# AlexandreRouma/SDRPlusPlus

Measured on AMD Instinct MI355X. Metric: IQ Msamples/s ingested (65536-pt FFT + 32 VFO WFM), higher is better.
Workload: dtype f32

## Files before the change

include/sdrpp_gpu.h:

```cpp
#ifndef SDRPP_GPU_H
#define SDRPP_GPU_H

#include <stddef.h>
#include <stdint.h>

#ifdef __cplusplus
extern "C" {
#endif

#define SDRPP_OK 0
#define SDRPP_ERR_NO_DEVICE (-1)
#define SDRPP_ERR_INVALID (-2)
#define SDRPP_ERR_NOMEM (-3)
#define SDRPP_ERR_HIP (-4)
#define SDRPP_ERR_UNSUPPORTED (-5)
#define SDRPP_ERR_NOT_FOUND (-6)

typedef struct sdrpp_ctx sdrpp_ctx;

int sdrpp_device_count(void);
int sdrpp_create(int device, int64_t max_push, sdrpp_ctx** ctx);
int sdrpp_destroy(sdrpp_ctx* ctx);
const char* sdrpp_strerror(int code);
const char* sdrpp_last_error(const sdrpp_ctx* ctx);
// ... 196 lines not shown
} sdrpp_iq_format;
int sdrpp_push_raw(sdrpp_ctx* ctx, const void* iq_host, int64_t count, const sdrpp_iq_format* fmt);
int sdrpp_push_frame(sdrpp_ctx* ctx, const unsigned char* frame, int bytes, int* samples);
int sdrpp_design_u8_table(int source, float gain, float* table256);
int sdrpp_abi_sizeof_iq_format(void);

void* sdrpp_host_alloc(size_t bytes);
void sdrpp_host_free(void* p);
void* sdrpp_device_alloc(sdrpp_ctx* ctx, size_t bytes);
void sdrpp_device_free(sdrpp_ctx* ctx, void* p);
int sdrpp_device_copy(sdrpp_ctx* ctx, void* dst, const void* src, size_t bytes, int kind);
int sdrpp_set_deferred(sdrpp_ctx* ctx, int on);
int sdrpp_push_pinned_async(sdrpp_ctx* ctx, const float* iq_pinned, int64_t count);
int sdrpp_push_wait(sdrpp_ctx* ctx);
int64_t sdrpp_pending(sdrpp_ctx* ctx);

int sdrpp_push_stage(sdrpp_ctx* ctx, int64_t count, float** slot);
int sdrpp_push_staged(sdrpp_ctx* ctx, int64_t count);
int sdrpp_push_staged_when(sdrpp_ctx* ctx, int64_t count, const volatile uint32_t* pending);
#define SDRPP_RESULT_SLOTS 24
#define SDRPP_GROUP_MAX 32
typedef struct sdrpp_result {
    uint64_t ticket;
    int n_vfo;
    const int* ids;
    const int64_t* offsets;
    const int* counts;
    const float* samples;
    int n_lines, fft_size, data_width;
    const float* zoomed;
    const int32_t* index;
    const float* raw;
    int n_iq;
    const float* iq;
} sdrpp_result;
int sdrpp_set_pipelined(sdrpp_ctx* ctx, int on, int result_flags);
int sdrpp_result_rec(sdrpp_ctx* ctx, uint64_t ticket, int id, const void** data, sdrpp_rec_info* info);
#define SDRPP_RESULT_RDS 32
int sdrpp_pipeline_set_rds_results(sdrpp_ctx* ctx, int on);
int sdrpp_result_rds(sdrpp_ctx* ctx, uint64_t ticket, int id, const float** data, int* count);
int sdrpp_result_meters(sdrpp_ctx* ctx, uint64_t ticket, const float** data, int* n_lines, int* n_meters);
int sdrpp_set_pipeline_group(sdrpp_ctx* ctx, int max_blocks, int adaptive);
int sdrpp_pipeline_launch_held(sdrpp_ctx* ctx);
int sdrpp_pipeline_group_stats(sdrpp_ctx* ctx, int64_t* out, int max);
uint64_t sdrpp_ticket(sdrpp_ctx* ctx);
int sdrpp_pipeline_flush(sdrpp_ctx* ctx);
int sdrpp_result_ready(sdrpp_ctx* ctx, uint64_t ticket);
int sdrpp_result_wait(sdrpp_ctx* ctx, uint64_t ticket, sdrpp_result* out);
int sdrpp_result_release(sdrpp_ctx* ctx, uint64_t ticket);
int sdrpp_result_take_lines(sdrpp_ctx* ctx, uint64_t ticket, float* zoomed_dst, int32_t* index_dst, int max_lines, int* n_lines);
#define SDRPP_PIPELINE_STATS_HEAD 8
int sdrpp_pipeline_stats(sdrpp_ctx* ctx, int64_t* out, int max);
const char* sdrpp_pipeline_role_name(int role);
int sdrpp_pass_form_stats(sdrpp_ctx* ctx, int64_t* out, const char** names, int max);

#define SDRPP_NUM_KERNEL_FAMILIES 13
int sdrpp_timing_enable(sdrpp_ctx* ctx, int on);
int sdrpp_timing_read(sdrpp_ctx* ctx, double* ms_per_family, int64_t* launches_per_family);
const char* sdrpp_kernel_family_name(int family);

#ifdef __cplusplus
}
#endif
#endif
```

sdrplusplus_amd/capi.py:

```python
import ctypes as C
import os

import numpy as np

_HERE = os.path.dirname(os.path.abspath(__file__))
DEFAULT_LIB = os.path.join(_HERE, "csrc", "libsdrpp_gpu.so")

MAX_DECIM_STAGES = 4
NUM_KERNEL_FAMILIES = 13

DEMOD_RAW, DEMOD_WFM, DEMOD_NFM, DEMOD_AM, DEMOD_USB, DEMOD_LSB, DEMOD_DSB, DEMOD_CW = -1, 0, 1, 2, 3, 4, 5, 6

c_float_p = C.POINTER(C.c_float)
c_int_p = C.POINTER(C.c_int)
c_int32_p = C.POINTER(C.c_int32)


class VfoDesc(C.Structure):

    _fields_ = [
        ("phase_delta_re", C.c_float),
        ("phase_delta_im", C.c_float),
        ("n_stages", C.c_int),
        ("stage_decim", C.c_int * MAX_DECIM_STAGES),
# ... 265 lines not shown
    L.sdrpp_vfo_remove.argtypes = [vp, C.c_int]
    L.sdrpp_vfo_replace.argtypes = [vp, C.c_int, C.POINTER(VfoDesc), C.c_int, c_int_p]
    L.sdrpp_vfo_count.argtypes = [vp]
    L.sdrpp_vfo_set_phase_delta.argtypes = [vp, C.c_int, C.c_float, C.c_float]
    L.sdrpp_vfo_set_channel_taps.argtypes = [vp, C.c_int, c_float_p, C.c_int]
    L.sdrpp_vfo_reset.argtypes = [vp, C.c_int]
    L.sdrpp_set_reference_block.argtypes = [vp, C.c_int]
    L.sdrpp_set_deferred.argtypes = [vp, C.c_int]
    L.sdrpp_push_pinned_async.argtypes = [vp, c_float_p, C.c_int64]
    L.sdrpp_push_wait.argtypes = [vp]
    L.sdrpp_push_stage.argtypes = [vp, C.c_int64, C.POINTER(c_float_p)]
    L.sdrpp_push_staged.argtypes = [vp, C.c_int64]
    L.sdrpp_push_staged_when.argtypes = [vp, C.c_int64, C.POINTER(C.c_uint32)]
    L.sdrpp_host_alloc.restype = vp
    L.sdrpp_host_alloc.argtypes = [C.c_size_t]
    L.sdrpp_host_free.restype = None
    L.sdrpp_host_free.argtypes = [vp]
    L.sdrpp_device_alloc.restype = vp
    L.sdrpp_device_alloc.argtypes = [vp, C.c_size_t]
    L.sdrpp_device_free.restype = None
    L.sdrpp_device_free.argtypes = [vp, vp]
    L.sdrpp_device_copy.restype = C.c_int
    L.sdrpp_device_copy.argtypes = [vp, vp, vp, C.c_size_t, C.c_int]
    L.sdrpp_pending.restype = C.c_int64
    L.sdrpp_pending.argtypes = [vp]
    L.sdrpp_vfo_read_many.argtypes = [vp, C.c_int, c_int_p, c_int_p, c_float_p, C.c_int64, C.POINTER(C.c_int64), c_int_p]
    L.sdrpp_set_nco_mode.argtypes = [vp, C.c_int]
    L.sdrpp_set_backend_pipeline.argtypes = [vp, C.c_int]
    L.sdrpp_vfo_set_ssb_phase_delta.argtypes = [vp, C.c_int, C.c_float, C.c_float]
    L.sdrpp_vfo_out_count.argtypes = [vp, C.c_int]
    L.sdrpp_vfo_read.argtypes = [vp, C.c_int, c_float_p, C.c_int]
    L.sdrpp_vfo_device_buffers.argtypes = [vp, C.c_int, C.POINTER(vp), c_int_p, C.POINTER(vp), c_int_p]
    L.sdrpp_push.argtypes = [vp, c_float_p, C.c_int64]
    L.sdrpp_push_device.argtypes = [vp, vp, C.c_int64]
    L.sdrpp_push_int16.argtypes = [vp, C.POINTER(C.c_int16), C.c_int64]
    L.sdrpp_abi_sizeof_iq_format.argtypes = []
    if L.sdrpp_abi_sizeof_iq_format() != C.sizeof(IqFormat):
        raise ImportError("sdrpp_iq_format layout mismatch: library %d bytes, binding %d" % (L.sdrpp_abi_sizeof_iq_format(), C.sizeof(IqFormat)))
    L.sdrpp_push_raw.argtypes = [vp, vp, C.c_int64, C.POINTER(IqFormat)]
    L.sdrpp_push_frame.argtypes = [vp, C.c_char_p, C.c_int, c_int_p]
    L.sdrpp_design_u8_table.argtypes = [C.c_int, C.c_float, c_float_p]
    L.sdrpp_set_pipelined.argtypes = [vp, C.c_int, C.c_int]
    L.sdrpp_set_pipeline_group.argtypes = [vp, C.c_int, C.c_int]
    L.sdrpp_pipeline_group_stats.argtypes = [vp, C.POINTER(C.c_int64), C.c_int]
    L.sdrpp_ticket.restype = C.c_uint64
    L.sdrpp_ticket.argtypes = [vp]
    L.sdrpp_pipeline_flush.argtypes = [vp]
    L.sdrpp_pipeline_launch_held.argtypes = [vp]
    L.sdrpp_result_ready.argtypes = [vp, C.c_uint64]
    L.sdrpp_result_wait.argtypes = [vp, C.c_uint64, C.POINTER(Result)]
    L.sdrpp_result_release.argtypes = [vp, C.c_uint64]
    L.sdrpp_result_take_lines.argtypes = [vp, C.c_uint64, vp, vp, C.c_int, c_int_p]
    L.sdrpp_pipeline_stats.argtypes = [vp, C.POINTER(C.c_int64), C.c_int]
    L.sdrpp_pipeline_role_name.restype = C.c_char_p
    L.sdrpp_pipeline_role_name.argtypes = [C.c_int]
    L.sdrpp_pass_form_stats.argtypes = [vp, C.POINTER(C.c_int64), C.POINTER(C.c_char_p), C.c_int]
    L.sdrpp_timing_enable.argtypes = [vp, C.c_int]
    L.sdrpp_timing_read.argtypes = [vp, C.POINTER(C.c_double), C.POINTER(C.c_int64)]
    L.sdrpp_kernel_family_name.restype = C.c_char_p
    L.sdrpp_kernel_family_name.argtypes = [C.c_int]
    _lib, _lib_path = L, path
    return L


EXPORTED_SYMBOLS = [
    "sdrpp_create", "sdrpp_destroy", "sdrpp_strerror", "sdrpp_last_error", "sdrpp_set_stream", "sdrpp_sync", "sdrpp_abi_version", "sdrpp_device_info",
    "sdrpp_design_low_pass", "sdrpp_design_high_pass", "sdrpp_design_fft_window", "sdrpp_design_reshape_params",
    "sdrpp_design_phase_delta", "sdrpp_design_resampler", "sdrpp_design_waterfall_view", "sdrpp_design_deemphasis_alpha",
    "sdrpp_vfo_read_pcm", "sdrpp_vfo_read_compressed", "sdrpp_preproc_read_pcm",
    "sdrpp_wf_configure", "sdrpp_wf_set_smoothing", "sdrpp_wf_set_hold", "sdrpp_wf_latest", "sdrpp_wf_raster", "sdrpp_wf_signal_info",
    "sdrpp_wf_set_meters", "sdrpp_wf_meters_read", "sdrpp_result_meters", "sdrpp_abi_sizeof_meter_desc",
    "sdrpp_preproc_configure", "sdrpp_preproc_reconfigure", "sdrpp_preproc_set_reference_order", "sdrpp_preproc_out_count", "sdrpp_preproc_read", "sdrpp_preproc_device_buffer",
    "sdrpp_vfo_set_rec", "sdrpp_vfo_rec_read", "sdrpp_abi_sizeof_rec_desc", "sdrpp_result_rec",
    "sdrpp_vfo_set_rds", "sdrpp_vfo_rds_count", "sdrpp_vfo_rds_read", "sdrpp_vfo_rds_device_buffer", "sdrpp_abi_sizeof_rds_desc", "sdrpp_rds_bank_count",
    "sdrpp_pipeline_set_rds_results", "sdrpp_result_rds",
    "sdrpp_vfo_set_stereo", "sdrpp_abi_sizeof_stereo_desc", "sdrpp_design_band_pass_complex", "sdrpp_design_pll",
    "sdrpp_vfo_set_af", "sdrpp_vfo_af_count", "sdrpp_vfo_af_read", "sdrpp_vfo_af_device_buffer", "sdrpp_abi_sizeof_af_desc",
    "sdrpp_vfo_set_if", "sdrpp_vfo_set_fmnr", "sdrpp_vfo_ifc_count", "sdrpp_vfo_ifc_read", "sdrpp_vfo_ifc_device_buffer", "sdrpp_abi_sizeof_if_desc",
    "sdrpp_fft_configure", "sdrpp_fft_disable", "sdrpp_fft_set_view", "sdrpp_fft_lines", "sdrpp_fft_read", "sdrpp_fft_copy_device", "sdrpp_fft_device_buffers",
    "sdrpp_vfo_add", "sdrpp_vfo_remove", "sdrpp_vfo_replace", "sdrpp_vfo_count", "sdrpp_vfo_set_phase_delta", "sdrpp_vfo_set_channel_taps", "sdrpp_vfo_reset",
    "sdrpp_vfo_out_count", "sdrpp_vfo_read", "sdrpp_vfo_device_buffers",
    "sdrpp_set_reference_block", "sdrpp_set_nco_mode", "sdrpp_set_backend_pipeline", "sdrpp_vfo_set_ssb_phase_delta", "sdrpp_vfo_read_many", "sdrpp_set_deferred", "sdrpp_push_pinned_async", "sdrpp_push_wait", "sdrpp_pending", "sdrpp_host_alloc", "sdrpp_host_free", "sdrpp_device_alloc", "sdrpp_device_free", "sdrpp_device_copy", "sdrpp_device_count",
    "sdrpp_push_raw", "sdrpp_push_frame", "sdrpp_design_u8_table", "sdrpp_abi_sizeof_iq_format",
    "sdrpp_push", "sdrpp_push_device", "sdrpp_push_int16", "sdrpp_push_stage", "sdrpp_push_staged", "sdrpp_push_staged_when",
    "sdrpp_set_pipelined", "sdrpp_set_pipeline_group", "sdrpp_pipeline_group_stats", "sdrpp_ticket", "sdrpp_pipeline_flush", "sdrpp_pipeline_launch_held", "sdrpp_result_ready", "sdrpp_result_wait", "sdrpp_result_release", "sdrpp_result_take_lines", "sdrpp_pipeline_stats", "sdrpp_pipeline_role_name", "sdrpp_pass_form_stats",
    "sdrpp_timing_enable", "sdrpp_timing_read", "sdrpp_kernel_family_name",
]


def pass_form_names():
    names = (C.c_char_p * 128)()
    n = load().sdrpp_pass_form_stats(None, None, names, 128)
    return [names[i].decode() for i in range(n)]


def design_low_pass(cutoff, trans_width, sample_rate, odd=False):
    L = load()
    n = L.sdrpp_design_low_pass(cutoff, trans_width, sample_rate, int(odd), None, 0)
    taps = np.zeros(max(n, 1), dtype=np.float32)
    L.sdrpp_design_low_pass(cutoff, trans_width, sample_rate, int(odd), taps.ctypes.data_as(c_float_p), n)
    return taps[:n]


def design_high_pass(cutoff, trans_width, sample_rate, odd=False):
    L = load()
    n = L.sdrpp_design_high_pass(cutoff, trans_width, sample_rate, int(odd), None, 0)
    taps = np.zeros(max(n, 1), dtype=np.float32)
    L.sdrpp_design_high_pass(cutoff, trans_width, sample_rate, int(odd), taps.ctypes.data_as(c_float_p), n)
    return taps[:n]


def design_band_pass_complex(band_start, band_stop, trans_width, sample_rate, odd=False):
    L = load()
    n = L.sdrpp_design_band_pass_complex(band_start, band_stop, trans_width, sample_rate, int(odd), None, 0)
    if n <= 0:
        raise SdrppError(n, "sdrpp_design_band_pass_complex")
    taps = np.empty(n, dtype=np.complex64)
    L.sdrpp_design_band_pass_complex(band_start, band_stop, trans_width, sample_rate, int(odd), taps.view(np.float32).ctypes.data_as(c_float_p), 2 * n)
    return taps


def design_pll(bandwidth):
    a, b = C.c_float(), C.c_float()
    load().sdrpp_design_pll(bandwidth, C.byref(a), C.byref(b))
    return a.value, b.value


def design_fft_window(kind, nz):
    w = np.empty(nz, dtype=np.float32)
    rc = load().sdrpp_design_fft_window(kind, nz, w.ctypes.data_as(c_float_p))
    if rc:
        raise SdrppError(rc, "bad window parameters")
    return w


def design_reshape_params(sample_rate, fft_size, fft_rate):
    skip, nz = C.c_int(), C.c_int()
    load().sdrpp_design_reshape_params(sample_rate, fft_size, fft_rate, C.byref(skip), C.byref(nz))
# ... 458 lines not shown
    def push_staged_from(self, iq):
        iq = np.ascontiguousarray(iq, dtype=np.complex64)
        slot = c_float_p()
        self._chk(self.L.sdrpp_push_stage(self.h, len(iq), C.byref(slot)))
        C.memmove(slot, iq.ctypes.data, len(iq) * 8)
        self._chk(self.L.sdrpp_push_staged(self.h, len(iq)))

    def push_staged_late_fill(self, iq, delay_s=0.002):
        import threading
        import time

        iq = np.ascontiguousarray(iq, dtype=np.complex64)
        slot = c_float_p()
        self._chk(self.L.sdrpp_push_stage(self.h, len(iq), C.byref(slot)))
        pending = C.c_uint32(2)
        dst = C.cast(slot, C.c_void_p).value
        half = (len(iq) // 2) * 8

        def fill():
            time.sleep(delay_s)
            C.memmove(dst, iq.ctypes.data, half)
            pending.value = 1
            time.sleep(delay_s)
            C.memmove(dst + half, iq.ctypes.data + half, len(iq) * 8 - half)
            pending.value = 0

        th = threading.Thread(target=fill)
        th.start()
        try:
            self._chk(self.L.sdrpp_push_staged_when(self.h, len(iq), C.byref(pending)))
        finally:
            th.join()

    def result_lines_into(self, ticket, dst_addr, max_lines):
        n = self._take_n
        rc = self.L.sdrpp_result_take_lines(self.h, ticket, dst_addr, None, max_lines, n)
        if rc < 0:
            self._chk(rc)
        return self._take_n_val.value

    def result_release(self, ticket):
        self._chk(self.L.sdrpp_result_release(self.h, int(ticket)))

    def pipeline_stats(self):
        buf = (C.c_int64 * 128)()
        n = self._chk(self.L.sdrpp_pipeline_stats(self.h, buf, 128))
        nroles = int(buf[5])
        roles = {}
        for r in range(nroles):
            if 8 + r < n and buf[8 + r]:
                roles[self.L.sdrpp_pipeline_role_name(r).decode()] = int(buf[8 + r])
        return dict(ticks=int(buf[0]), tick_blocks=int(buf[1]), pass_blocks=int(buf[2]), crowded_ticks=int(buf[3]), depth=int(buf[4]), table_bytes=int(buf[7]), roles=roles)

    def pass_form_stats(self):
        buf = (C.c_int64 * 128)()
        names = (C.c_char_p * 128)()
        n = self._chk(self.L.sdrpp_pass_form_stats(self.h, buf, names, 128))
        return {names[i].decode(): int(buf[i]) for i in range(n) if buf[i]}

    def timing_enable(self, on=True, families=None):
        v = int(bool(on))
        if on and families is not None:
            mask = 0
            for f in families:
                mask |= 1 << int(f)
            v = (1 | (mask << 1)) if mask else 0
        self._chk(self.L.sdrpp_timing_enable(self.h, v))

    def family_index(self, name):
        for i in range(NUM_KERNEL_FAMILIES):
            if self.L.sdrpp_kernel_family_name(i).decode() == name:
                return i
        raise KeyError(name)

    def timing_read(self):
        ms = (C.c_double * NUM_KERNEL_FAMILIES)()
        ln = (C.c_int64 * NUM_KERNEL_FAMILIES)()
        self._chk(self.L.sdrpp_timing_read(self.h, ms, ln))
        return {self.L.sdrpp_kernel_family_name(i).decode(): (ms[i], ln[i]) for i in range(NUM_KERNEL_FAMILIES)}


_hip = None


def _copy_from_device(L, host_ptr, dev_ptr, nbytes):
    global _hip
    if "emu" in os.path.basename(lib_path()):
        C.memmove(host_ptr, dev_ptr, nbytes)
        return
    if _hip is None:
        _hip = C.CDLL("libamdhip64.so")
        _hip.hipMemcpy.argtypes = [C.c_void_p, C.c_void_p, C.c_size_t, C.c_int]
    rc = _hip.hipMemcpy(C.c_void_p(host_ptr), C.c_void_p(dev_ptr), nbytes, 2)
    if rc:
        raise SdrppError(-4, "hipMemcpy D2H failed (%d)" % rc)
```

sdrplusplus_amd/csrc/host_ctx.h:

```cpp
#pragma once

namespace {

constexpr int kArenaSlots = 24;
constexpr size_t kArenaBytes = 4u << 20;
constexpr int kRing = 4;
constexpr int kTickDepth = 18;
constexpr int kResSlots = SDRPP_RESULT_SLOTS;
constexpr int kGroupMax = SDRPP_GROUP_MAX;
constexpr int kResMeta = kResSlots * kGroupMax;
constexpr int kStageSlots = 4;
constexpr int kChanMaxTaps = 65536;
constexpr int kAfHpfMaxTaps = 65536;
constexpr int kFmifTile = SDRPP_FMIF_TILE;
constexpr int kFmifSeg = SDRPP_FMIF_SEG;
constexpr size_t kScratchBytes = 64u << 20;
constexpr int kMaxLds = 64 * 1024;

enum Family { F_FFT1 = 0, F_FFT2, F_FFTS, F_ZOOM, F_S1, F_DECIM, F_POLY, F_FIR, F_DEMOD, F_MISC, F_AF, F_PIPE, F_TICK };
const char* kFamilyNames[SDRPP_NUM_KERNEL_FAMILIES] = { "fft_pass1", "fft_pass2", "fft_single", "zoom_palette", "vfo_stage1",
                                                        "vfo_decim", "vfo_poly",  "vfo_fir",    "demod",        "carry_misc", "af_chain",  "vfo_pipe", "tick" };

struct Stream {
    int width = 2;
// ... 340 lines not shown
    uint64_t pushes = 0;
    uint64_t land_tick = 0;
    TickTable* next_tab = nullptr;
    int next_tab_n = 0;
    TickTable* empty_tab = nullptr;
    unsigned* d_tick_counter = nullptr;
    unsigned tick_target = 0;
    unsigned* h_tick_flag = nullptr;
    unsigned* hd_tick_flag = nullptr;
    uint64_t arena_tick[kArenaSlots] = {};
    float* tick_land[3] = {};
    std::vector<float> tick_land_tab[3];
    float* stage_host[kStageSlots] = {};
    uint64_t stage_tick[kStageSlots] = {};
    int stage_cur = 0;
    int stage_open = -1;
    char* res_ring = nullptr;
    char* res_ring_dev = nullptr;
    size_t res_ring_bytes = 0;
    size_t res_cap = 0;
    size_t res_head = 0;
    int res_epoch = 0;
    struct ResRegion { uint64_t gid; size_t off, bytes; int held; };
    std::deque<ResRegion> res_live;
    struct ResRetired { char* ring; int epoch; int held; };
    std::vector<ResRetired> res_retired;
    Result res[kResMeta];
    int group_max = 1;
    int group_adaptive = 0;
    bool stage_pend_stable = false;
    struct Held {
        int kind = -1;
        int fmt_type = 0;
        float fmt_scalar = 0.0f;
        std::vector<float> fmt_table;
        const char* base = nullptr;
        int stage_slot = -1;
        int64_t total = 0;
        std::vector<int> ends;
    } held;
    std::vector<int> grp_ends;
    int64_t plan_fft_pos0 = 0, plan_fft_next0 = 0;
    uint64_t groups = 0;
    int64_t stat_groups = 0, stat_group_blocks = 0, stat_group_max = 0;
    static constexpr int kTickEvents = 32;
    hipEvent_t tick_ev[kTickEvents] = {};
    uint64_t tick_ev_tick[kTickEvents] = {};
    hipEvent_t tick_ev_start[kTickEvents] = {};
    int tick_ev_next = 0;
    uint64_t tick_ev_last = 0;
    void* bank_plan = nullptr;
    void (*bank_plan_free)(void*) = nullptr;
    int64_t stat_tick_blocks = 0, stat_pass_blocks = 0, stat_crowded = 0, stat_last_depth = 0, stat_last_table_bytes = 0;
    int64_t stat_role_wgs[64] = {};
    int64_t stat_pass_forms[96] = {};

    bool timing = false;
    unsigned timing_mask = 0xffffffffu;
    std::vector<TimingPair> tpairs;
    std::vector<hipEvent_t> ev_pool;
    double fam_ms[SDRPP_NUM_KERNEL_FAMILIES] = {};
    int64_t fam_launch[SDRPP_NUM_KERNEL_FAMILIES] = {};
};
```

sdrplusplus_amd/csrc/sdrpp_gpu.hip:

```cpp
#include <hip/hip_runtime.h>
#include <hip/hip_ext.h>

#include <algorithm>
#include <chrono>
#include <atomic>
#include <cmath>
#include <cstdarg>
#include <cstdio>
#include <cstring>
#include <deque>
#include <map>
#include <memory>
#include <mutex>
#include <string>
#include <thread>
#include <vector>

#include "../../include/sdrpp_gpu.h"
#include "fft_kernels.h"
#include "host_design.h"
#include "vfo_kernels.h"
#include "pipe_kernels.h"
#include "tick_kernels.h"

// ... 1611 lines not shown
    if (data) { *data = R->n_lines > 0 ? reinterpret_cast<const float*>(R->base + R->off_meters) : nullptr; }
    if (n_lines) { *n_lines = R->n_lines; }
    if (n_meters) { *n_meters = R->n_meters; }
    return SDRPP_OK;
}
int sdrpp_result_release(sdrpp_ctx* c, uint64_t ticket) {
    if (!c || ticket == 0 || ticket > c->pushes) { return c ? SDRPP_ERR_NOT_FOUND : SDRPP_ERR_INVALID; }
    sdrpp_ctx::Result& R = c->res[ticket % kResMeta];
    if (R.ticket != ticket) { return SDRPP_ERR_NOT_FOUND; }
    if (R.held) {
        if (sdrpp_ctx::ResRegion* g = tick_results_region(c, R.group)) {
            if (g->held > 0) { g->held--; }
        }
        if (R.epoch != c->res_epoch) {
            for (size_t i = 0; i < c->res_retired.size(); i++) {
                if (c->res_retired[i].epoch == R.epoch && --c->res_retired[i].held <= 0) {
                    DeviceScope dev_scope_(c);
                    (void)hipHostFree(c->res_retired[i].ring);
                    c->res_retired.erase(c->res_retired.begin() + (long)i);
                    break;
                }
            }
        }
    }
    R.held = false;
    R.ticket = 0;
    return SDRPP_OK;
}

int sdrpp_result_take_lines(sdrpp_ctx* c, uint64_t ticket, float* zoomed_dst, int32_t* index_dst, int max_lines, int* n_lines) {
    sdrpp_result r{};
    int rc = sdrpp_result_wait(c, ticket, &r);
    if (rc) { return rc; }
    if (n_lines) { *n_lines = r.n_lines; }
    if (r.n_lines > max_lines) {
        (void)sdrpp_result_release(c, ticket);
        return fail(c, SDRPP_ERR_INVALID, "block %llu completed %d lines, room for %d", (unsigned long long)ticket, r.n_lines, max_lines);
    }
    if (r.n_lines > 0 && r.zoomed) {
        const size_t bytes = (size_t)r.n_lines * (size_t)r.data_width * 4;
        if (zoomed_dst) { memcpy(zoomed_dst, r.zoomed, bytes); }
        if (index_dst) { memcpy(index_dst, r.index, bytes); }
    }
    return sdrpp_result_release(c, ticket);
}
int sdrpp_pipeline_stats(sdrpp_ctx* c, int64_t* out, int max) {
    if (!c || !out || max < 0) { return SDRPP_ERR_INVALID; }
    const int64_t head[SDRPP_PIPELINE_STATS_HEAD] = { (int64_t)c->ticks, c->stat_tick_blocks, c->stat_pass_blocks, c->stat_crowded, c->stat_last_depth, (int64_t)TR_COUNT, 0, c->stat_last_table_bytes };
    int n = 0;
    for (; n < SDRPP_PIPELINE_STATS_HEAD && n < max; n++) { out[n] = head[n]; }
    for (int r = 0; r < TR_COUNT && n < max; r++, n++) { out[n] = c->stat_role_wgs[r]; }
    return n;
}
const char* sdrpp_pipeline_role_name(int role) {
    static const char* const names[] = { "none", "copy", "carry", "rot", "fcm_132_4", "fcm_6", "fcm_10", "fcm_16", "fcm16_132_4", "fcl_0", "fcl_pf", "toep_c", "toep_r", "toep_q",
                                         "firb_c", "firb_r", "firb_s", "firb_q", "pre", "seq", "fft_s10", "fft_s11", "fft_s12", "fft_p1_5", "fft_p1_6", "fft_p1_7", "fft_p1_8", "fft_p1_9",
                                         "fft_p1_10", "fft_p2_7", "fft_p2_8", "fft_p2_9", "fft_p2_10", "fft_p2row", "fft_tr", "zoom_16", "zoom_4", "zoom_1", "polyc", "deemp_p0", "deemp_p1",
                                         "dc_p0", "dc_p1", "wf_ring", "wf_trace", "pipe", "rotx16", "fird", "ssbx", "s1_1", "s1d_1", "f2_1", "poly", "ifc" };
    static_assert(sizeof(names) / sizeof(names[0]) == TR_COUNT, "role names out of step with TickRole");
    return (role >= 0 && role < TR_COUNT) ? names[role] : nullptr;
}
int sdrpp_pass_form_stats(sdrpp_ctx* c, int64_t* out, const char** names, int max) {
    static const char* const extra[] = { "polyb_4", "polyb_8", "polyb_4_odd", "polyb_8_odd", "s1_8", "s1_4", "s1_2", "s1d_8", "s1d_4", "s1d_2", "f2_8_44_3", "f2_8", "f2_4", "f2_2", "rotx_1" };
    static_assert(sizeof(extra) / sizeof(extra[0]) == PF_COUNT - TR_COUNT, "form names out of step with PassForm");
    if (max < 0 || (out && !c)) { return SDRPP_ERR_INVALID; }
    int n = 0;
    for (; n < PF_COUNT && n < max; n++) {
        if (out) { out[n] = c->stat_pass_forms[n]; }
        if (names) { names[n] = n < TR_COUNT ? sdrpp_pipeline_role_name(n) : extra[n - TR_COUNT]; }
    }
    return n;
}

int sdrpp_timing_enable(sdrpp_ctx* c, int on) {
    DeviceScope dev_scope_(c);
    if (!c) { return SDRPP_ERR_INVALID; }
    timing_flush(c);
    c->timing = on != 0;
    c->timing_mask = (on > 1) ? (unsigned)(on >> 1) : 0xffffffffu;
    for (int i = 0; i < SDRPP_NUM_KERNEL_FAMILIES; i++) {
        c->fam_ms[i] = 0.0;
        c->fam_launch[i] = 0;
    }
    return SDRPP_OK;
}

int sdrpp_timing_read(sdrpp_ctx* c, double* ms, int64_t* launches) {
    DeviceScope dev_scope_(c);
    if (!c) { return SDRPP_ERR_INVALID; }
    timing_flush(c);
    for (int i = 0; i < SDRPP_NUM_KERNEL_FAMILIES; i++) {
        if (ms) { ms[i] = c->fam_ms[i]; }
        if (launches) { launches[i] = c->fam_launch[i]; }
    }
    return SDRPP_OK;
}

}
```

sdrplusplus_amd/csrc/tick_host.h:

```cpp
#pragma once

namespace {

void tick_wait_done(sdrpp_ctx* c, uint64_t nticks) {
    if (!c->h_tick_flag) { return; }
    const volatile unsigned* f = c->h_tick_flag;
    long spins = 0;
    while ((int)((unsigned)nticks - *f) > 0) {
        if (++spins > 2000) { std::this_thread::yield(); }
        if (spins > 40000000) {
            (void)hipStreamSynchronize(c->stream);
            if ((int)((unsigned)nticks - *f) > 0) { return; }
        }
    }
}
hipEvent_t tick_event_take(sdrpp_ctx* c, uint64_t behind_tick) {
    const int k = c->tick_ev_next;
    c->tick_ev_next = (k + 1) % sdrpp_ctx::kTickEvents;
    tick_ev_resolve(c, k);
    if (!c->tick_ev[k] && hipEventCreate(&c->tick_ev[k]) != hipSuccess) { return nullptr; }
    c->tick_ev_tick[k] = behind_tick;
    c->tick_ev_last = behind_tick;
    return c->tick_ev[k];
}
// ... 64 lines not shown
        T->n = (int)nx.size();
        int total = 0;
        for (size_t i = 0; i < nx.size(); i++) {
            total += nx[i].e.gx * nx[i].e.gy;
            T->block_end[i] = total;
            T->e[i] = nx[i].e;
        }
        c->arena_off = off + offsetof(TickTable, e) + nx.size() * sizeof(TickEntry);
        tab_dev_next = reinterpret_cast<TickTable*>(c->arena_dev + off);
        tab_n_next = (int)nx.size();
    }
    TickL0 l0{};
    if (land && land->bytes > 0) {
        l0.job[0] = *land;
        l0.blocks[0] = (int)std::max<long long>(1, std::min<long long>((land->bytes + 8191) / 8192, c->tick_land_blocks));
        if ((land->kind & 0xff) == 4) { l0.blocks[0] = (int)std::max<long long>(1, std::min<long long>(land->bytes / 32768, c->tick_land_blocks)); }
    }
    if (c->arena_off > 0) {
        l0.job[1] = CopyJob{ c->arena_host_dev[c->arena_slot], c->arena_dev, (long long)((c->arena_off + 15) & ~(size_t)15), 0, 0 };
        l0.blocks[1] = (int)std::max<size_t>(1, std::min<size_t>((c->arena_off + 4095) / 4096, 16));
    }
    int blocks = l0.blocks[0] + l0.blocks[1];
    size_t lds = 0;
    bool set1 = false;
    long long role_wgs = 0;
    bool to_host = false;
    for (auto& r : now) {
        to_host = to_host || r.to_host;
        blocks += r.e.gx * r.e.gy;
        role_wgs += (long long)r.e.gx * r.e.gy;
        lds = std::max(lds, r.lds);
        set1 = set1 || r.e.role == TR_FCL_PF || r.e.role == TR_FCM_6 || r.e.role == TR_FCM_10 || r.e.role == TR_FCM_16;
        if (r.e.role >= 0 && r.e.role < 64) { c->stat_role_wgs[r.e.role] += (int64_t)r.e.gx * r.e.gy; }
    }
    if (role_wgs > 3ll * c->num_cus) { c->stat_crowded++; }
    {
        const int l0_at = c->tick_l0_at;
        const int role_blocks = blocks - l0.blocks[0] - l0.blocks[1];
        l0.first = l0_at < 0 ? role_blocks : std::min(l0_at, role_blocks);
    }
    if (blocks == 0) {
        c->next_tab = tab_dev_next;
        c->next_tab_n = tab_n_next;
        for (auto& R : c->res) {
            if (R.ticket != 0 && R.done_tick > c->ticks) { R.done_tick--; }
        }
        return SDRPP_OK;
    }
    c->tick_target += (unsigned)blocks;
    c->ticks++;
    TickDone done{ c->d_tick_counter, c->hd_tick_flag, c->tick_target, (unsigned)c->ticks };
    hipEvent_t stop_ev = nullptr;
    const TickTable* tab = c->next_tab_n > 0 ? c->next_tab : c->empty_tab;
    {
        const bool timed = c->timing && ((c->timing_mask >> F_TICK) & 1u);
        c->fam_launch[F_TICK]++;
        hipEvent_t ea = nullptr;
        if (timed || to_host) {
            const int k = c->tick_ev_next;
            stop_ev = tick_event_take(c, c->ticks);
            if (!stop_ev) { return fail(c, SDRPP_ERR_HIP, "hipEventCreate failed"); }
            if (timed) {
                ea = get_event(c);
                c->tick_ev_start[k] = ea;
            }
        }
        HostScope hs("launch");
        if (stop_ev) {
            if (set1) { hipExtLaunchKernelGGL((tick_kernel<1>), dim3((unsigned)blocks), dim3(256), (unsigned)lds, c->stream, ea, stop_ev, 0, l0, tab, done); }
            else { hipExtLaunchKernelGGL((tick_kernel<0>), dim3((unsigned)blocks), dim3(256), (unsigned)lds, c->stream, ea, stop_ev, 0, l0, tab, done); }
        }
        else if (set1) { hipLaunchKernelGGL((tick_kernel<1>), dim3((unsigned)blocks), dim3(256), lds, c->stream, l0, tab, done); }
        else { hipLaunchKernelGGL((tick_kernel<0>), dim3((unsigned)blocks), dim3(256), lds, c->stream, l0, tab, done); }
    }
    c->arena_tick[c->arena_slot] = c->ticks;
    c->next_tab = tab_dev_next;
    c->next_tab_n = tab_n_next;
    hipError_t e = hipGetLastError();
    if (e != hipSuccess) { return fail(c, SDRPP_ERR_HIP, "tick launch failed: %s", hipGetErrorString(e)); }
    return SDRPP_OK;
}
int tick_drain(sdrpp_ctx* c) {
    while (!c->tickq.empty()) {
        int rc = arena_begin(c);
        if (rc) { return rc; }
        rc = tick_launch(c, nullptr);
        if (rc) { return rc; }
    }
    return SDRPP_OK;
}

bool tick_eligible(sdrpp_ctx* c) {
    if ((c->pre.on && c->pre.ref_order) || c->deferred) { return false; }
    for (auto& kv : c->vfos) {
        const Vfo& v = *kv.second;
        if ((v.nco_exact && c->rot_exact_single) || !v.recs.empty() || v.st.size() > 24) { return false; }
    }
    return true;
}

const Stream& result_stream(const Vfo& v, int* level = nullptr) {
    if (v.af.on && v.af.i_last >= 0 && v.d.demod != SDRPP_DEMOD_RAW) {
        if (level) { *level = v.lvl_af; }
        return v.st[(size_t)v.af.i_last];
    }
    const bool raw = v.d.demod == SDRPP_DEMOD_RAW;
// ... 617 lines not shown
```

sdrplusplus_amd/csrc/vfo_ifchain_kernels.h:

```cpp
#pragma once
#include <hip/hip_runtime.h>
#include <stdint.h>
#include <sdrpp_gfx950.h>

namespace sdrpp_k {

enum WaveKind : int { WK_NBSQ, WK_FMIF, WK_RDS_FRONT, WK_RDS_ROTX, WK_RDS_LINE, WK_ST_PILOT, WK_ST_LOOP, WK_ST_MATRIX, WK_COUNT };
struct WaveJob {
    const void* rec;
    int kind;
    int arg;
};
static_assert(sizeof(WaveJob) == 16, "the role's table: 16 bytes per wavefront");
constexpr bool wave_kind_uses_lds(int kind) { return kind == WK_FMIF || kind == WK_RDS_FRONT || kind == WK_ST_PILOT || kind == WK_ST_LOOP || kind == WK_ST_MATRIX; }

template <class T>
__device__ __forceinline__ const T* wave_uniform_ptr(const T* p) {
    const uint64_t a = (uint64_t)(uintptr_t)p;
    const uint32_t lo = (uint32_t)wave_uniform((int)(uint32_t)a), hi = (uint32_t)wave_uniform((int)(uint32_t)(a >> 32));
    return reinterpret_cast<const T*>((uintptr_t)(((uint64_t)hi << 32) | (uint64_t)lo));
}
template <class T>
__device__ __forceinline__ T wave_uniform_job(const T* p) {
    static_assert(sizeof(T) % 4 == 0, "job records are whole words");
    const UniformI32 u = as_uniform_i32(wave_uniform_ptr(p));
    int w[sizeof(T) / 4];
#pragma unroll
    for (int i = 0; i < (int)(sizeof(T) / 4); i++) { w[i] = u[i]; }
    T job;
    __builtin_memcpy(&job, w, sizeof(T));
    return job;
}

}

#define SDRPP_WAVE_LDS_FLOATS ((SDRPP_FMIF_SEG + SDRPP_FMIF_TILE) * 2 + 64 * 4)
#include "vfo_fmif_kernels.h"
#include "vfo_rds_kernels.h"
#include "vfo_stereo_kernels.h"

namespace sdrpp_k {

static_assert(SDRPP_FMIF_LDS_FLOATS <= SDRPP_WAVE_LDS_FLOATS, "FMIF: window and exchange");
static_assert(SDRPP_ST_PILOT_TILE + SDRPP_ST_PILOT_MAX_TAPS <= SDRPP_WAVE_LDS_FLOATS, "stereo pilot: phases of a tile and the taps in front of it");
static_assert(2 * (SDRPP_ST_MATRIX_TILE + SDRPP_ST_AUDIO_MAX_TAPS - 1) <= SDRPP_WAVE_LDS_FLOATS, "stereo matrix: two windows");
static_assert(SDRPP_ST_LOOP_PTRS + SDRPP_ST_LOOP_CHUNK + SDRPP_ST_PACK <= SDRPP_WAVE_LDS_FLOATS, "stereo loop: the rows of a chunk");

struct NbSqJob {
    const float2* in;
    float2* out;
    float* amp;
    int n;
    int nb_on;
    float nb_rate, nb_inv_rate, nb_level;
    int sq_on;
    float sq_level;
    const int* bounds;
    int nb;
};
__device__ __forceinline__ void vfo_nbsq_body(const NbSqJob& job) {
    const int lane = threadIdx.x & 63;
    const int nblk = job.bounds ? job.nb : 1;
    float amp = job.nb_on ? *job.amp : 1.0f;
    int blk_lo = 0;
    for (int blk = 0; blk < nblk; blk++) {
        const int n = job.bounds ? job.bounds[blk] : job.n;
        float part = 0.0f;
        if (!job.nb_on) {
            constexpr int U = 4;
            for (int base = blk_lo; base < n; base += 64 * U) {
                float2 xv[U];
#pragma unroll
                for (int u = 0; u < U; u++) {
                    const int i = base + 64 * u + lane;
                    xv[u] = (i < n) ? job.in[i] : make_float2(0.0f, 0.0f);
                }
#pragma unroll
                for (int u = 0; u < U; u++) {
                    const int i = base + 64 * u + lane;
                    if (i < n) {
                        part += sqrtf((xv[u].x * xv[u].x) + (xv[u].y * xv[u].y));
                        job.out[i] = xv[u];
                    }
                }
            }
// ... 62 lines not shown
```

sdrplusplus_amd/csrc/vfo_toep_kernels.h:

```cpp
#pragma once
#include <hip/hip_runtime.h>
#include <stdint.h>
#include <sdrpp_gfx950.h>
#include "fft_kernels.h"
#include "vfo_stream.h"
#include "vfo_fir_kernels.h"

namespace sdrpp_k {

struct ToepJob {
    StreamIn in;
    float* out;
    const float* tl;
    const int* lbase;
    int tl_len, nsteps;
    int s_in, rows;
    int base0;
    int nout;
    int mt_per_wave;
    float inv_deviation;
};

#ifdef SDRPP_TOEP_KNOCK
__device__ int g_toep_knock;
#endif
#ifdef SDRPP_TOEP_PROF
__device__ unsigned long long g_toep_prof[4][8];
#define TOEP_TICK() ((long long)__builtin_readcyclecounter())
#endif

template <int WIDTH, int G, bool QUAD>
__device__ __forceinline__ void vfo_toep_body(const KIdx bid, const KIdx gdim, float* smemt, const ToepJob* __restrict__ jobs) {
    const ToepJob job = jobs[bid.y];
    const int tid = threadIdx.x, lane = tid & 63, wv = tid >> 6;
#ifdef SDRPP_TOEP_KNOCK
    const int knock = g_toep_knock;
#endif
    const int nsteps = job.nsteps, s_in = job.s_in, rows = job.rows;
    const int span = (G * 16 - 1) * s_in + 4 * nsteps;
    const int pl = (span + 8) & ~3;
    constexpr int NPL = (WIDTH == 2 || QUAD) ? 2 : 1;
    const int tl_pad = (job.tl_len + 3) & ~3;
    float* TLs = smemt;
    float* XR = smemt + tl_pad + wv * NPL * pl;
    float* XI = XR + pl;
    {
        constexpr int NB = 4;
        for (int i0 = tid; i0 < job.tl_len; i0 += 256 * NB) {
            float tv[NB];
#pragma unroll
            for (int q = 0; q < NB; q++) { tv[q] = global_load_f32(job.tl, min(i0 + q * 256, job.tl_len - 1)); }
#pragma unroll
            for (int q = 0; q < NB; q++) {
                if (i0 + q * 256 < job.tl_len) { TLs[i0 + q * 256] = tv[q]; }
            }
        }
    }
    __syncthreads();
    TICK_MARK(0);
    const int omt = G * 16 * rows;
    const int mt0 = bid.x * 4 + wv, mts = gdim.x * 4;
    const int c = lane & 15, kk = lane >> 4;
    const float* Bp = TLs + global_load_i32(job.lbase, lane);
    const float* Ar = XR + c * s_in + kk;
    const float* Ai = XI + c * s_in + kk;
    constexpr bool ILV = (WIDTH == 2) && !QUAD;
    float2* X2 = reinterpret_cast<float2*>(XR);
    const float2* A2 = X2 + c * s_in + kk;
    constexpr int PF = 18;
    constexpr int PF4 = 9;
    constexpr bool CPLX_IN = (WIDTH == 2) || QUAD;
    const int cnt = QUAD ? span + 1 : span;
    const int npair = (cnt + 1) >> 1;
    const bool piped = ILV ? (npair <= PF4 * 64) : (cnt <= PF * 64);
    float2 pf2[(CPLX_IN && !ILV) ? PF : 1];
    float pf1[CPLX_IN ? 1 : PF];
    float4 pf4[ILV ? PF4 : 1];
    auto fetch = [&](int mt) {
#ifdef SDRPP_TOEP_KNOCK
        if (knock & 2) { return; }
#endif
        const int lo = job.base0 + mt * G * 16 * s_in - (QUAD ? 1 : 0);
        const bool inside = lo >= 0 && lo + cnt <= job.in.n;
        if constexpr (ILV) {
            if (inside) {
#pragma unroll
                for (int q = 0; q < PF4; q++) {
                    const int e = q * 64 + lane;
                    pf4[q] = (e < npair) ? global_load_f32x4_unaligned(job.in.data, 2ll * (lo + 2 * e)) : make_float4(0.0f, 0.0f, 0.0f, 0.0f);
                }
            }
            else {
#pragma unroll
                for (int q = 0; q < PF4; q++) {
                    const int e = q * 64 + lane;
                    const float2 a = stream_load2_nb(job.in, lo + 2 * e, e < npair), b = stream_load2_nb(job.in, lo + 2 * e + 1, e < npair);
                    pf4[q] = make_float4(a.x, a.y, b.x, b.y);
                }
            }
        }
        else if constexpr (CPLX_IN) {
            if (inside) {
                const float2* src2 = reinterpret_cast<const float2*>(job.in.data) + lo;
#pragma unroll
                for (int q = 0; q < PF; q++) {
                    const int s = q * 64 + lane;
                    pf2[q] = (s < cnt) ? global_load_f32x2(src2, s) : make_float2(0.0f, 0.0f);
                }
            }
            else {
#pragma unroll
                for (int q = 0; q < PF; q++) {
                    const int s = q * 64 + lane;
                    pf2[q] = stream_load2_nb(job.in, lo + s, s < cnt);
                }
            }
        }
        else {
            if (inside) {
#pragma unroll
                for (int q = 0; q < PF; q++) {
                    const int s = q * 64 + lane;
                    pf1[q] = (s < cnt) ? global_load_f32(job.in.data + lo, s) : 0.0f;
                }
            }
            else {
#pragma unroll
                for (int q = 0; q < PF; q++) {
                    const int s = q * 64 + lane;
                    pf1[q] = stream_load1_nb(job.in, lo + s, s < cnt);
                }
            }
        }
    };
    auto window_store = [&]() {
        if constexpr (ILV) {
            float4* X4 = reinterpret_cast<float4*>(XR);
#pragma unroll
            for (int q = 0; q < PF4; q++) {
                const int e = q * 64 + lane;
                if (e < npair) { X4[e] = pf4[q]; }
            }
            return;
        }
#pragma unroll
        for (int q = 0; q < PF; q++) {
            const int s = q * 64 + lane;
            if (s < cnt) {
                if constexpr (QUAD) { XI[s] = fm_phase(pf2[q].y, pf2[q].x); }
                else if constexpr (WIDTH == 2) {
                    XR[s] = pf2[q].x;
                    XI[s] = pf2[q].y;
                }
                else { XR[s] = pf1[q]; }
            }
        }
    };
    auto discriminate = [&]() {
        if constexpr (QUAD) {
            wave_sync();
            for (int s = lane; s < span; s += 64) { XR[s] = normalize_phase(XI[s + 1] - XI[s]) * job.inv_deviation; }
        }
    };
#ifdef SDRPP_TOEP_PROF
    long long tp_acc[5] = { 0, 0, 0, 0, 0 }, tp_rounds = 0;
    const long long tp_birth = TOEP_TICK();
#endif
    if (piped && mt0 * omt < job.nout) {
        fetch(mt0);
        window_store();
        if (1 < job.mt_per_wave && (mt0 + mts) * omt < job.nout) { fetch(mt0 + mts); }
        discriminate();
        TICK_MARK(1);
    }
    for (int it = 0; it < job.mt_per_wave; it++) {
        const int mt = mt0 + it * mts;
        const int obase = mt * omt;
        if (obase >= job.nout) { break; }
        if (!piped) {
            const int lo = job.base0 + mt * G * 16 * s_in - (QUAD ? 1 : 0);
            for (int s = lane; s < cnt; s += 64) {
                if constexpr (QUAD) {
                    const float2 x = stream_load2(job.in, lo + s);
                    XI[s] = fm_phase(x.y, x.x);
                }
                else if constexpr (WIDTH == 2) { X2[s] = stream_load2(job.in, lo + s); }
                else { XR[s] = stream_load1(job.in, lo + s); }
            }
            discriminate();
        }
        wave_sync();
#ifdef SDRPP_TOEP_PROF
        const long long tp0 = TOEP_TICK();
#endif
        f32x4 accR[G], accI[G];
#pragma unroll
        for (int g = 0; g < G; g++) { accR[g] = mfma4_zero(); accI[g] = mfma4_zero(); }
        {
            constexpr int U = (WIDTH == 2) ? 4 : 8;
            int t0 = 0;
#ifdef SDRPP_TOEP_KNOCK
            if (knock & 4) { t0 = nsteps; }
#endif
            for (; t0 + U <= nsteps; t0 += U) {
                float b[U], xr[U][G], xi[U][G];
#pragma unroll
                for (int u = 0; u < U; u++) {
                    b[u] = Bp[4 * (t0 + u)];
#pragma unroll
                    for (int g = 0; g < G; g++) {
                        if constexpr (ILV) {
                            const float2 a = A2[g * 16 * s_in + 4 * (t0 + u)];
                            xr[u][g] = a.x;
                            xi[u][g] = a.y;
                        }
                        else {
                            xr[u][g] = Ar[g * 16 * s_in + 4 * (t0 + u)];
                            if constexpr (WIDTH == 2) { xi[u][g] = Ai[g * 16 * s_in + 4 * (t0 + u)]; }
                        }
                    }
                }
#pragma unroll
                for (int u = 0; u < U; u++) {
#pragma unroll
// ... 105 lines not shown
```

Baseline: 24340.

## Overlap Toeplitz tap-table staging with first window fetch; load job wave-uniformly

The Toeplitz VFO kernel now issues the first input-window fetch (and its store, plus the prefetch of the second tile) while the tap table is still being copied into LDS. The block barrier moves after those steps, so the global-load latency of the taps and of the input window overlap instead of running back to back. The job record is also read through a wave-uniform scalar-load helper, moved into a shared header, to cut per-lane vector loads. It also adds a small stat API reporting the tick table entry count. The reordering raises register pressure from holding the prefetch and tap values at the same time.

After: 24490, median of 6. No clear change (+0.6%).

```diff
diff --git a/include/sdrpp_gpu.h b/include/sdrpp_gpu.h
--- a/include/sdrpp_gpu.h
+++ b/include/sdrpp_gpu.h
@@ -272,6 +272,7 @@
 #define SDRPP_PIPELINE_STATS_HEAD 8
 int sdrpp_pipeline_stats(sdrpp_ctx* ctx, int64_t* out, int max);
 const char* sdrpp_pipeline_role_name(int role);
+int sdrpp_pipeline_tick_entries(sdrpp_ctx* ctx);
 int sdrpp_pass_form_stats(sdrpp_ctx* ctx, int64_t* out, const char** names, int max);
 
 #define SDRPP_NUM_KERNEL_FAMILIES 13
diff --git a/sdrplusplus_amd/capi.py b/sdrplusplus_amd/capi.py
--- a/sdrplusplus_amd/capi.py
+++ b/sdrplusplus_amd/capi.py
@@ -341,6 +341,7 @@
     L.sdrpp_result_release.argtypes = [vp, C.c_uint64]
     L.sdrpp_result_take_lines.argtypes = [vp, C.c_uint64, vp, vp, C.c_int, c_int_p]
     L.sdrpp_pipeline_stats.argtypes = [vp, C.POINTER(C.c_int64), C.c_int]
+    L.sdrpp_pipeline_tick_entries.argtypes = [vp]
     L.sdrpp_pipeline_role_name.restype = C.c_char_p
     L.sdrpp_pipeline_role_name.argtypes = [C.c_int]
     L.sdrpp_pass_form_stats.argtypes = [vp, C.POINTER(C.c_int64), C.POINTER(C.c_char_p), C.c_int]
@@ -372,7 +373,7 @@
     "sdrpp_set_reference_block", "sdrpp_set_nco_mode", "sdrpp_set_backend_pipeline", "sdrpp_vfo_set_ssb_phase_delta", "sdrpp_vfo_read_many", "sdrpp_set_deferred", "sdrpp_push_pinned_async", "sdrpp_push_wait", "sdrpp_pending", "sdrpp_host_alloc", "sdrpp_host_free", "sdrpp_device_alloc", "sdrpp_device_free", "sdrpp_device_copy", "sdrpp_device_count",
     "sdrpp_push_raw", "sdrpp_push_frame", "sdrpp_design_u8_table", "sdrpp_abi_sizeof_iq_format",
     "sdrpp_push", "sdrpp_push_device", "sdrpp_push_int16", "sdrpp_push_stage", "sdrpp_push_staged", "sdrpp_push_staged_when",
-    "sdrpp_set_pipelined", "sdrpp_set_pipeline_group", "sdrpp_pipeline_group_stats", "sdrpp_ticket", "sdrpp_pipeline_flush", "sdrpp_pipeline_launch_held", "sdrpp_result_ready", "sdrpp_result_wait", "sdrpp_result_release", "sdrpp_result_take_lines", "sdrpp_pipeline_stats", "sdrpp_pipeline_role_name", "sdrpp_pass_form_stats",
+    "sdrpp_set_pipelined", "sdrpp_set_pipeline_group", "sdrpp_pipeline_group_stats", "sdrpp_ticket", "sdrpp_pipeline_flush", "sdrpp_pipeline_launch_held", "sdrpp_result_ready", "sdrpp_result_wait", "sdrpp_result_release", "sdrpp_result_take_lines", "sdrpp_pipeline_stats", "sdrpp_pipeline_tick_entries", "sdrpp_pipeline_role_name", "sdrpp_pass_form_stats",
     "sdrpp_timing_enable", "sdrpp_timing_read", "sdrpp_kernel_family_name",
 ]
 
@@ -937,6 +938,9 @@
                 roles[self.L.sdrpp_pipeline_role_name(r).decode()] = int(buf[8 + r])
         return dict(ticks=int(buf[0]), tick_blocks=int(buf[1]), pass_blocks=int(buf[2]), crowded_ticks=int(buf[3]), depth=int(buf[4]), table_bytes=int(buf[7]), roles=roles)
 
+    def pipeline_tick_entries(self):
+        return self._chk(self.L.sdrpp_pipeline_tick_entries(self.h))
+
     def pass_form_stats(self):
         buf = (C.c_int64 * 128)()
         names = (C.c_char_p * 128)()
diff --git a/sdrplusplus_amd/csrc/host_ctx.h b/sdrplusplus_amd/csrc/host_ctx.h
--- a/sdrplusplus_amd/csrc/host_ctx.h
+++ b/sdrplusplus_amd/csrc/host_ctx.h
@@ -416,6 +416,7 @@
     void* bank_plan = nullptr;
     void (*bank_plan_free)(void*) = nullptr;
     int64_t stat_tick_blocks = 0, stat_pass_blocks = 0, stat_crowded = 0, stat_last_depth = 0, stat_last_table_bytes = 0;
+    int stat_last_entries = 0;
     int64_t stat_role_wgs[64] = {};
     int64_t stat_pass_forms[96] = {};
 
diff --git a/sdrplusplus_amd/csrc/sdrpp_gpu.hip b/sdrplusplus_amd/csrc/sdrpp_gpu.hip
--- a/sdrplusplus_amd/csrc/sdrpp_gpu.hip
+++ b/sdrplusplus_amd/csrc/sdrpp_gpu.hip
@@ -1687,6 +1687,10 @@
     for (int r = 0; r < TR_COUNT && n < max; r++, n++) { out[n] = c->stat_role_wgs[r]; }
     return n;
 }
+int sdrpp_pipeline_tick_entries(sdrpp_ctx* c) {
+    if (!c) { return SDRPP_ERR_INVALID; }
+    return c->stat_last_entries;
+}
 const char* sdrpp_pipeline_role_name(int role) {
     static const char* const names[] = { "none", "copy", "carry", "rot", "fcm_132_4", "fcm_6", "fcm_10", "fcm_16", "fcm16_132_4", "fcl_0", "fcl_pf", "toep_c", "toep_r", "toep_q",
                                          "firb_c", "firb_r", "firb_s", "firb_q", "pre", "seq", "fft_s10", "fft_s11", "fft_s12", "fft_p1_5", "fft_p1_6", "fft_p1_7", "fft_p1_8", "fft_p1_9",
diff --git a/sdrplusplus_amd/csrc/tick_host.h b/sdrplusplus_amd/csrc/tick_host.h
--- a/sdrplusplus_amd/csrc/tick_host.h
+++ b/sdrplusplus_amd/csrc/tick_host.h
@@ -140,6 +140,7 @@
     TickDone done{ c->d_tick_counter, c->hd_tick_flag, c->tick_target, (unsigned)c->ticks };
     hipEvent_t stop_ev = nullptr;
     const TickTable* tab = c->next_tab_n > 0 ? c->next_tab : c->empty_tab;
+    c->stat_last_entries = c->next_tab_n;
     {
         const bool timed = c->timing && ((c->timing_mask >> F_TICK) & 1u);
         c->fam_launch[F_TICK]++;
diff --git a/sdrplusplus_amd/csrc/vfo_ifchain_kernels.h b/sdrplusplus_amd/csrc/vfo_ifchain_kernels.h
--- a/sdrplusplus_amd/csrc/vfo_ifchain_kernels.h
+++ b/sdrplusplus_amd/csrc/vfo_ifchain_kernels.h
@@ -2,6 +2,7 @@
 #include <hip/hip_runtime.h>
 #include <stdint.h>
 #include <sdrpp_gfx950.h>
+#include "vfo_uniform.h"
 
 namespace sdrpp_k {
 
@@ -13,24 +14,6 @@
 };
 static_assert(sizeof(WaveJob) == 16, "the role's table: 16 bytes per wavefront");
 constexpr bool wave_kind_uses_lds(int kind) { return kind == WK_FMIF || kind == WK_RDS_FRONT || kind == WK_ST_PILOT || kind == WK_ST_LOOP || kind == WK_ST_MATRIX; }
-
-template <class T>
-__device__ __forceinline__ const T* wave_uniform_ptr(const T* p) {
-    const uint64_t a = (uint64_t)(uintptr_t)p;
-    const uint32_t lo = (uint32_t)wave_uniform((int)(uint32_t)a), hi = (uint32_t)wave_uniform((int)(uint32_t)(a >> 32));
-    return reinterpret_cast<const T*>((uintptr_t)(((uint64_t)hi << 32) | (uint64_t)lo));
-}
-template <class T>
-__device__ __forceinline__ T wave_uniform_job(const T* p) {
-    static_assert(sizeof(T) % 4 == 0, "job records are whole words");
-    const UniformI32 u = as_uniform_i32(wave_uniform_ptr(p));
-    int w[sizeof(T) / 4];
-#pragma unroll
-    for (int i = 0; i < (int)(sizeof(T) / 4); i++) { w[i] = u[i]; }
-    T job;
-    __builtin_memcpy(&job, w, sizeof(T));
-    return job;
-}
 
 }
 
diff --git a/sdrplusplus_amd/csrc/vfo_toep_kernels.h b/sdrplusplus_amd/csrc/vfo_toep_kernels.h
--- a/sdrplusplus_amd/csrc/vfo_toep_kernels.h
+++ b/sdrplusplus_amd/csrc/vfo_toep_kernels.h
@@ -5,6 +5,7 @@
 #include "fft_kernels.h"
 #include "vfo_stream.h"
 #include "vfo_fir_kernels.h"
+#include "vfo_uniform.h"
 
 namespace sdrpp_k {
 
@@ -31,7 +32,7 @@
 
 template <int WIDTH, int G, bool QUAD>
 __device__ __forceinline__ void vfo_toep_body(const KIdx bid, const KIdx gdim, float* smemt, const ToepJob* __restrict__ jobs) {
-    const ToepJob job = jobs[bid.y];
+    const ToepJob job = wave_uniform_job(jobs + bid.y);
     const int tid = threadIdx.x, lane = tid & 63, wv = tid >> 6;
 #ifdef SDRPP_TOEP_KNOCK
     const int knock = g_toep_knock;
@@ -44,24 +45,10 @@
     float* TLs = smemt;
     float* XR = smemt + tl_pad + wv * NPL * pl;
     float* XI = XR + pl;
-    {
-        constexpr int NB = 4;
-        for (int i0 = tid; i0 < job.tl_len; i0 += 256 * NB) {
-            float tv[NB];
-#pragma unroll
-            for (int q = 0; q < NB; q++) { tv[q] = global_load_f32(job.tl, min(i0 + q * 256, job.tl_len - 1)); }
-#pragma unroll
-            for (int q = 0; q < NB; q++) {
-                if (i0 + q * 256 < job.tl_len) { TLs[i0 + q * 256] = tv[q]; }
-            }
-        }
-    }
-    __syncthreads();
-    TICK_MARK(0);
     const int omt = G * 16 * rows;
     const int mt0 = bid.x * 4 + wv, mts = gdim.x * 4;
     const int c = lane & 15, kk = lane >> 4;
-    const float* Bp = TLs + global_load_i32(job.lbase, lane);
+    const int lb_lane = global_load_i32(job.lbase, lane);
     const float* Ar = XR + c * s_in + kk;
     const float* Ai = XI + c * s_in + kk;
     constexpr bool ILV = (WIDTH == 2) && !QUAD;
@@ -166,10 +153,29 @@
     long long tp_acc[5] = { 0, 0, 0, 0, 0 }, tp_rounds = 0;
     const long long tp_birth = TOEP_TICK();
 #endif
-    if (piped && mt0 * omt < job.nout) {
-        fetch(mt0);
+    const bool own = piped && mt0 * omt < job.nout;
+    {
+        constexpr int NB = 4;
+        for (int s0 = 0; s0 < job.tl_len; s0 += 256 * NB) {
+            const int i0 = s0 + tid;
+            float tv[NB];
+#pragma unroll
+            for (int q = 0; q < NB; q++) { tv[q] = global_load_f32(job.tl, min(i0 + q * 256, job.tl_len - 1)); }
+            if (s0 == 0 && own) { fetch(mt0); }
+#pragma unroll
+            for (int q = 0; q < NB; q++) {
+                if (i0 + q * 256 < job.tl_len) { TLs[i0 + q * 256] = tv[q]; }
+            }
+        }
+    }
+    if (own) {
         window_store();
         if (1 < job.mt_per_wave && (mt0 + mts) * omt < job.nout) { fetch(mt0 + mts); }
+    }
+    __syncthreads();
+    TICK_MARK(0);
+    const float* Bp = TLs + lb_lane;
+    if (own) {
         discriminate();
         TICK_MARK(1);
     }
diff --git a/sdrplusplus_amd/csrc/vfo_uniform.h b/sdrplusplus_amd/csrc/vfo_uniform.h
--- /dev/null
+++ b/sdrplusplus_amd/csrc/vfo_uniform.h
@@ -0,0 +1,26 @@
+#pragma once
+#include <hip/hip_runtime.h>
+#include <stdint.h>
+#include <sdrpp_gfx950.h>
+
+namespace sdrpp_k {
+
+template <class T>
+__device__ __forceinline__ const T* wave_uniform_ptr(const T* p) {
+    const uint64_t a = (uint64_t)(uintptr_t)p;
+    const uint32_t lo = (uint32_t)wave_uniform((int)(uint32_t)a), hi = (uint32_t)wave_uniform((int)(uint32_t)(a >> 32));
+    return reinterpret_cast<const T*>((uintptr_t)(((uint64_t)hi << 32) | (uint64_t)lo));
+}
+template <class T>
+__device__ __forceinline__ T wave_uniform_job(const T* p) {
+    static_assert(sizeof(T) % 4 == 0, "job records are whole words");
+    const UniformI32 u = as_uniform_i32(wave_uniform_ptr(p));
+    int w[sizeof(T) / 4];
+#pragma unroll
+    for (int i = 0; i < (int)(sizeof(T) / 4); i++) { w[i] = u[i]; }
+    T job;
+    __builtin_memcpy(&job, w, sizeof(T));
+    return job;
+}
+
+}
```
